# jmschrei/PyPore

Measured on AMD Instinct MI355X. Metric: Msamples/sec segmented (SpeedyStatSplit, 10^8-sample trace); %HBM roofline, higher is better.
Workload: dtype int32/f64 (exact integer block sums of fp32 or int16 samples; decisions in fp64)

## Files before the change

### pypore_amd/csrc/poreseg.hip

```cpp
#include <hip/hip_runtime.h>

#include <algorithm>
#include <chrono>
#include <complex>
#include <cmath>
#include <cstdarg>
#include <cstdio>
#include <cstdlib>
#include <cstring>
#include <condition_variable>
#include <mutex>
#include <string>
#include <thread>
#include <tuple>
#include <vector>

#include "poreseg.h"
#include "seg_device.hpp"
#include "seg_align.hpp"
#include "seg_pairwise.hpp"
#include "seg_hmm.hpp"

using namespace ps;

// ... 150 lines not shown
    }
    return code;
}

#define HIP_TRY(ctx, expr)                                                                        \
    do {                                                                                          \
        hipError_t e_ = (expr);                                                                   \
        if (e_ != hipSuccess)                                                                     \
            return fail(ctx, PS_ERR_HIP, "%s failed: %s (%s:%d)", #expr, hipGetErrorString(e_), __FILE__, __LINE__); \
    } while (0)

struct FrontStream { std::mutex mu; hipStream_t s = nullptr; };
FrontStream g_front[16];
FrontStream *front_for(ps_ctx *ctx)
{
    if (ctx->device < 0 || ctx->device >= 16) return nullptr;
    FrontStream *f = &g_front[ctx->device];
    std::lock_guard<std::mutex> lk(f->mu);
    if (!f->s) {
#ifdef PS_DIAG
        int lo = 0, hi = 0;
        const char *pr = std::getenv("PORESEG_FRONT_PRIORITY");
        if (pr && std::atoi(pr) != 0 && hipDeviceGetStreamPriorityRange(&lo, &hi) == hipSuccess) {
            if (hipStreamCreateWithPriority(&f->s, hipStreamNonBlocking, hi) != hipSuccess) { f->s = nullptr; (void)hipGetLastError(); }
        }
#endif
        if (!f->s && hipStreamCreateWithFlags(&f->s, hipStreamNonBlocking) != hipSuccess) { f->s = nullptr; (void)hipGetLastError(); return nullptr; }
    }
    return f;
}

struct K0Chain {
    static constexpr int RING = 64;
    std::mutex mu;
    hipEvent_t ev[RING] = {};
    unsigned long long gen[RING];
    unsigned long long next = 0;
    bool made = false;
};
K0Chain g_chain[16];
int chain_enter(ps_ctx *ctx, int device, int max_in_flight, hipStream_t st, unsigned long long *ticket)
{
    K0Chain &c = g_chain[device & 15];
    std::lock_guard<std::mutex> lk(c.mu);
    if (!c.made) {
        for (int i = 0; i < K0Chain::RING; ++i) { HIP_TRY(ctx, hipEventCreateWithFlags(&c.ev[i], hipEventDisableTiming)); c.gen[i] = 0; }
        c.made = true;
    }
    const unsigned long long t = c.next++;
    *ticket = t;
    const int m = std::min(max_in_flight, K0Chain::RING / 2);
    if (t >= static_cast<unsigned long long>(m)) {
        const unsigned long long w = t - static_cast<unsigned long long>(m);
        if (c.gen[w % K0Chain::RING] == w + 1) HIP_TRY(ctx, hipStreamWaitEvent(st, c.ev[w % K0Chain::RING], 0));
    }
    return PS_OK;
}
int chain_publish(ps_ctx *ctx, int device, hipStream_t st, unsigned long long ticket)
{
    K0Chain &c = g_chain[device & 15];
    std::lock_guard<std::mutex> lk(c.mu);
    HIP_TRY(ctx, hipEventRecord(c.ev[ticket % K0Chain::RING], st));
    c.gen[ticket % K0Chain::RING] = ticket + 1;
    return PS_OK;
}
constexpr size_t SMALL_TAIL = 64 * 1024;
struct SmallLayout { unsigned long long status, work0, work1, work2, dense, stamp[12], life[9], qctl, qhead, tree_tail; AsmHeader hdr;
                     unsigned long long lat_ctl[6]; int lat_prog[LAT_D];
                     unsigned long long nt_cur; };

int make_cfg(ps_ctx *ctx, const void *d_samples, const ps_sample_format *fmt, int mw, int maxw, int W,
             double min_gain, DevCfg *c)
{
    if (!fmt) return fail(ctx, PS_ERR_ARG, "sample format is NULL");
    if (fmt->dtype != PS_DTYPE_F32 && fmt->dtype != PS_DTYPE_I16)
        return fail(ctx, PS_ERR_ARG, "unknown dtype %d", fmt->dtype);
    if (!(fmt->quantum > 0) || !std::isfinite(fmt->quantum))
        return fail(ctx, PS_ERR_ARG, "quantum must be positive and finite");
    c->samples = d_samples;
    c->dtype = fmt->dtype;
    c->off_counts = fmt->dtype == PS_DTYPE_F32 ? 0 : fmt->offset_counts;
    c->dc_counts = fmt->dtype == PS_DTYPE_F32 ? static_cast<double>(fmt->offset_counts) : 0.0;
    c->noise_k = ctx->noise_k;
    c->inv_q = static_cast<float>(1.0 / fmt->quantum);
    c->q = fmt->quantum;
    c->q2 = fmt->quantum * fmt->quantum;
    c->mw = mw; c->maxw = maxw; c->W = W; c->half = W / 2;
    c->min_gain = min_gain;
    c->mode = ctx->mode;
    c->prune = ctx->prune;
    c->lds_cap = std::max(1, std::min(W, ctx->lds_max_samples));
    c->bsum = nullptr; c->ev_info = nullptr; c->chunk_tot = nullptr; c->blk_mm = nullptr; c->grp = nullptr; c->bs_wide = 0;
    c->blk_cls = nullptr; c->cls_mm = nullptr; c->cls_kthr = 0;
    c->k0_unaligned = ctx->k0_unaligned;
    c->pre_c = nullptr; c->pre_c2 = nullptr;
    c->dbg = ctx->small.as<SmallLayout>()->stamp;
    c->nt_log = nullptr;
// ... 761 lines not shown
                                       ctx->bridges.as<int2>(), ctx->bmeta.as<int4>(), reinterpret_cast<unsigned *>(&sm->status),           \
                                       &sm->work0, static_cast<int>(n_ext), ctx->ext_list.as<int>(), ctx->bridge_ext.as<int2>(),           \
                                       ctx->ext_slot.as<int>(), slots_used, BR_MAX, ext_stride)
            if (wide) { if (f32) PS_EXT(PS_DTYPE_F32 | DT_WIDE); else PS_EXT(PS_DTYPE_I16 | DT_WIDE); }
            else      { if (f32) PS_EXT(PS_DTYPE_F32); else PS_EXT(PS_DTYPE_I16); }
#undef PS_EXT
            HIP_TRY(ctx, hipGetLastError());
        }
        ctx->counters[4] += static_cast<int64_t>(n_ext);
        slots_used += static_cast<int>(n_ext);
        items_cap += static_cast<int64_t>(n_ext) * ext_stride;
        const int64_t ts2 = total_len / mw + items_cap + 1;
        HIP_TRY(ctx, ctx->spine_items.reserve(static_cast<size_t>(items_cap) * sizeof(int4)));
        HIP_TRY(ctx, ctx->tree_jobs.reserve(static_cast<size_t>(items_cap) * sizeof(TreeJob)));
        HIP_TRY(ctx, ctx->tree_counts.reserve((static_cast<size_t>(items_cap) + (static_cast<size_t>(items_cap) >> GS_LOG) + 2) * sizeof(int32_t)));
        HIP_TRY(ctx, ctx->items.reserve(static_cast<size_t>(items_cap) * sizeof(Item)));
        HIP_TRY(ctx, ctx->item_pos.reserve((static_cast<size_t>(items_cap) + 1) * sizeof(int64_t)));
        HIP_TRY(ctx, ctx->tree_scratch.reserve(static_cast<size_t>(ts2) * sizeof(int32_t)));
        HIP_TRY(ctx, ctx->tree_spill.reserve(static_cast<size_t>(ts2) * sizeof(int2)));
    }
    ctx->counters[3] = hd.n_items;
    float ms = 0;
    if (ctx->timing >= 2 && nj && hipEventElapsedTime(&ms, ctx->ev[7], ctx->ev[0]) == hipSuccess) ctx->ms[6] = ms;
    if (ctx->timing >= 2 && nj && hipEventElapsedTime(&ms, ctx->ev[0], ctx->ev[6]) == hipSuccess) ctx->ms[0] = ms;
    if (ctx->timing >= 2 && nj && hipEventElapsedTime(&ms, ctx->ev[6], ctx->ev[1]) == hipSuccess) ctx->ms[5] = ms;
    if (ctx->timing >= 2 && hipEventElapsedTime(&ms, ctx->ev[1], ctx->ev[5]) == hipSuccess) ctx->ms[4] = ms;
    return rc;
}
int device_stitch_batch(ps_ctx *ctx, const DevCfg &cfg_in, int bs_mode, const int64_t *ev_start, const int64_t *ev_len, int32_t n_ev, int mw, int W,
                        int32_t *d_bounds, int64_t cap, int64_t *h_bounds_off, ps_segstat *d_stats,
                        std::chrono::steady_clock::time_point t_begin, bool digest_ready = false)
{
    const int rc = device_stitch_batch_(ctx, cfg_in, bs_mode, ev_start, ev_len, n_ev, mw, W, d_bounds, cap, h_bounds_off, d_stats, t_begin, digest_ready);
    ctx->chain_held = false;
    return rc;
}
}

namespace {
std::mutex g_probe_mu;
int g_unaligned_ok[16] = {-1, -1, -1, -1, -1, -1, -1, -1, -1, -1, -1, -1, -1, -1, -1, -1};
int k0_unaligned_probe(int device, hipStream_t st)
{
    std::lock_guard<std::mutex> lk(g_probe_mu);
    int &ok = g_unaligned_ok[device & 15];
    if (ok >= 0) return ok;
    ok = 0;
    unsigned char h[128];
    for (int i = 0; i < 128; ++i) h[i] = static_cast<unsigned char>(37 * i + 11);
    unsigned char *d = nullptr;
    unsigned *bad = nullptr;
    if (hipMalloc(&d, 256) != hipSuccess || hipMalloc(&bad, sizeof(unsigned)) != hipSuccess) { if (d) (void)hipFree(d); (void)hipGetLastError(); return ok; }
    unsigned hb = 1;
    if (hipMemcpyAsync(d, h, 128, hipMemcpyHostToDevice, st) == hipSuccess && hipMemsetAsync(bad, 0, sizeof(unsigned), st) == hipSuccess) {
        hipLaunchKernelGGL(k0_unaligned_probe_kernel<2>, dim3(1), dim3(64), 0, st, d, 16, bad);
        hipLaunchKernelGGL(k0_unaligned_probe_kernel<4>, dim3(1), dim3(64), 0, st, d, 16, bad);
        if (hipGetLastError() == hipSuccess && hipMemcpyAsync(&hb, bad, sizeof(unsigned), hipMemcpyDeviceToHost, st) == hipSuccess &&
            hipStreamSynchronize(st) == hipSuccess)
            ok = hb == 0 ? 1 : 0;
    }
    (void)hipFree(d); (void)hipFree(bad); (void)hipGetLastError();
    return ok;
}
}

#ifdef PS_DIAG
// ... 125 lines not shown
        ctx->n_cu = hipGetDeviceProperties(&prop, ctx->device) == hipSuccess ? prop.multiProcessorCount : 256;
    }
    HIP_TRY(ctx, hipStreamSynchronize(*st));
    HIP_TRY(ctx, hipStreamDestroy(*st));
    *st = nullptr;
    if (count <= 0) { HIP_TRY(ctx, hipStreamCreateWithFlags(st, hipStreamNonBlocking)); return PS_OK; }
    const int words = (ctx->n_cu + 31) / 32;
    std::vector<uint32_t> mask(static_cast<size_t>(words), invert ? 0xffffffffu : 0u);
    for (int k = 0; k < count; ++k) {
        const int b = first + k * std::max(1, stride);
        if (b < 0 || b >= ctx->n_cu) continue;
        if (invert) mask[b >> 5] &= ~(1u << (b & 31)); else mask[b >> 5] |= 1u << (b & 31);
    }
    if (ctx->n_cu & 31) mask[words - 1] &= (1u << (ctx->n_cu & 31)) - 1u;
    HIP_TRY(ctx, hipExtStreamCreateWithCUMask(st, static_cast<uint32_t>(words), mask.data()));
    return PS_OK;
}
#endif

int ps_set_option(ps_ctx *ctx, const char *name, int64_t value)
{
    if (!ctx || !name) return PS_ERR_ARG;
    const std::string n(name);
    if (n == "mode" && value >= 0 && value <= 2) ctx->mode = static_cast<int>(value);
    else if (n == "stitch_host") ctx->stitch_host = value != 0;
    else if (n == "prune") ctx->prune = value != 0;
    else if (n == "scan_bs") ctx->scan_bs = value != 0;
    else if (n == "near_tie_log" && value >= 0 && value <= (int64_t(1) << 30)) ctx->nt_cap = value;
    else if (n == "groups") ctx->groups = value != 0;
    else if (n == "tree_par") ctx->tree_par = value != 0;
    else if (n == "k0_waves" && value >= 0 && value <= 16) ctx->k0_waves = static_cast<int>(value);
    else if (n == "k0_shared") ctx->k0_shared = value != 0;
    else if (n == "k0_admit" && value >= 0) ctx->k0_admit = static_cast<int>(value);
    else if (n == "bridge_ext" && (value == 0 || value == 1)) ctx->bridge_ext_on = static_cast<int>(value);
    else if (n == "lat_help" && value >= 0 && value <= 2) ctx->lat_help = static_cast<int>(value);
    else if (n == "shared_device" && value >= 0 && value <= 4096) {
        const bool sh = value > 1;
        ctx->k0_waves = sh ? 1 : 0;
        ctx->lat_help = sh ? 0 : 1;
        ctx->k0_admit = value > 3 ? 3 : 0;
    }
    else if (n == "hmm_bp_budget" && value >= 1) ctx->hmm_bp_budget = value;
    else if (n == "hmm_fb_budget" && value >= 1) ctx->hmm_fb_budget = value;
    else if (n == "pairwise_budget" && value >= 1) ctx->pw_budget = value;
    else if (n == "hmm_expect_lds") ctx->hmm_expect_lds = value != 0;
    else if (n == "single_pass") ctx->single_pass = value != 0;
    else if (n == "gather_fused") ctx->gather_fused = value != 0;
    else if (n == "download_by_kernel") ctx->download_by_kernel = value != 0;
    else if (n == "debug") ctx->debug = value != 0;
    else if (n == "k0_unaligned") ctx->k0_unaligned = value != 0 ? k0_unaligned_probe(ctx->device, ctx->stream) : 0;
    else if (n == "slots_pct" && value >= 1 && value <= 100) ctx->slots_pct = static_cast<int>(value);
    else if (n == "tree_jobs_per_wave" && value >= 0 && value <= 1024) ctx->tree_jobs_per_wave = static_cast<int>(value);
    else if (n == "noise_k_ppm" && value >= 0) ctx->noise_k = static_cast<float>(static_cast<double>(value) * 1.0e-6);
#ifdef PS_DIAG
    else if (n == "dbg_phase" && value >= 0 && value <= 2) ctx->dbg_phase = static_cast<int>(value);
    else if (n == "dbg_k0_nogrp") ctx->dbg_k0_nogrp = value != 0;
    else if (n == "cu_mask" && ctx->own_stream)
        return diag_mask_stream(ctx, &ctx->stream, static_cast<int>(value & 0xfff), static_cast<int>((value >> 12) & 0xfff),
                                static_cast<int>((value >> 24) & 0xff), ((value >> 32) & 1) != 0);
    else if (n == "k0_sets" && value >= 2 && value <= 4) ctx->k0_sets = static_cast<int>(value);
    else if (n == "scan_lds_pad" && value >= 0 && value <= 65536) ctx->scan_lds_pad = static_cast<int>(value);
    else if (n == "rep_eval" && value >= 1) ctx->rep_eval = static_cast<int>(value);
    else if (n == "rep_stage" && value >= 1) ctx->rep_stage = static_cast<int>(value);
    else if (n == "rep_sum" && value >= 1) ctx->rep_sum = static_cast<int>(value);
#endif
    else if (n == "bridge_budget" && value >= 1 && value <= BR_MAX) ctx->bridge_budget = static_cast<int>(value);
// ... 671 lines not shown
        kk = std::max(-2147483000.0, std::min(2147483000.0, kk));
        long long k = static_cast<long long>(kk);
        while (k > -2147483000LL && !(static_cast<double>(k - 1) * q < threshold)) --k;
        while (k < 2147483000LL && static_cast<double>(k) * q < threshold) ++k;
        kthr = static_cast<int>(k);
    }
    hipLaunchKernelGGL(trace_setup_kernel, dim3(1), dim3(256), 0, ctx->stream, reinterpret_cast<unsigned long long *>(ctx->small.p),
                       static_cast<int>(sizeof(SmallLayout) / sizeof(unsigned long long)), ctx->det_cand.as<long long>(),
                       static_cast<long long>(n), static_cast<long long>(nb_total));
    HIP_TRY(ctx, hipGetLastError());
    cfg.grp = ctx->groups ? ctx->grp.p : nullptr;
    cfg.blk_mm = d_stats ? ctx->blk_mm.as<int>() : nullptr;
    cfg.blk_cls = ctx->blk_cls.as<unsigned char>();
    cfg.cls_mm = ctx->cls_mm.as<int2>();
    cfg.cls_kthr = kthr;
    if (ctx->n_cu <= 0) {
        hipDeviceProp_t prop;
        ctx->n_cu = hipGetDeviceProperties(&prop, ctx->device) == hipSuccess ? prop.multiProcessorCount : 256;
    }
    {
        const unsigned k0_full = static_cast<unsigned>((nb_pad / K0_WB + K0_WAVES - 1) / K0_WAVES);
        const unsigned k0_per_cu = static_cast<unsigned>(ctx->k0_waves) * (f32 ? 1u : 2u);
        const unsigned k0_grid = ctx->k0_waves > 0 ? std::min(k0_full, k0_per_cu * static_cast<unsigned>(ctx->n_cu) * (4u / K0_WAVES)) : k0_full;
        const int64_t *d_ev = ctx->det_cand.as<int64_t>();
        if (ctx->k0_admit > 0) {
            const int grc = chain_enter(ctx, ctx->device, ctx->k0_admit, ctx->stream, &ctx->chain_ticket);
            if (grc) return grc;
        }
#define PS_K0T(DTV) hipLaunchKernelGGL((blocksum_kernel<DTV, 2>), dim3(k0_grid), dim3(64 * K0_WAVES), 0, ctx->stream, cfg, d_ev, d_ev + 1, d_ev + 2, 1, n, \
                                     ctx->bsum.p, ctx->ev_info.as<int4>(), ctx->chunk_mabs.as<int4>(), reinterpret_cast<unsigned *>(&sm->status),          \
                                     const_cast<uint4 *>(static_cast<const uint4 *>(cfg.grp)))
        if (f32) PS_K0T(PS_DTYPE_F32); else PS_K0T(PS_DTYPE_I16);
#undef PS_K0T
        HIP_TRY(ctx, hipGetLastError());
        if (ctx->k0_admit > 0) { const int crc = chain_publish(ctx, ctx->device, ctx->stream, ctx->chain_ticket); if (crc) return crc; }
    }
    std::vector<int> tics;
    unsigned st = 0;
    rc = detect_edges(ctx, cfg, n, threshold, true, tics, &st);
    if (rc) return rc;
    if (st & ST_WIDE_RANGE) { ctx->counters[7] = 3; const int r2 = two_calls(); ctx->counters[7] = 3; return r2; }
    rc = events_from_edges(ctx, cfg, n, tics, threshold, min_duration, min_current, h_starts, h_lengths, ev_cap, n_events_out);
    if (rc) return rc;
    const int32_t n_ev = static_cast<int32_t>(*n_events_out);
    if (n_ev == 0) { ctx->nt_seen = 0; return PS_OK; }
    for (int e = 0; e < n_ev; ++e)
        if (h_lengths[e] > 0x7fffffff - 2LL * W - 16) return fail(ctx, PS_ERR_ARG, "event %d length %lld out of range", e, static_cast<long long>(h_lengths[e]));
    cfg.bsum = ctx->bsum.p;
    cfg.blk_cls = nullptr;
    rc = device_stitch_batch(ctx, cfg, 1, h_starts, h_lengths, n_ev, mw, W, d_bounds, cap, h_bounds_off, d_stats, t_begin, true);
    if (rc == RC_FALLBACK || rc == RC_WIDE) {
        return ps_segment_events(ctx, d_samples, fmt, h_starts, h_lengths, n_ev, params, d_bounds, cap, h_bounds_off, d_stats, nullptr);
    }
    if (rc == PS_OK) nt_keep(ctx, h_starts, h_lengths, n_ev);
    else ctx->nt_seen = -1;
    return rc;
}

int ps_get_near_ties(const ps_ctx *ctx, ps_near_tie *out, int32_t cap, int64_t *n_out)
{
    if (!ctx || !n_out || cap < 0 || (cap > 0 && !out)) return PS_ERR_ARG;
    if (ctx->nt_seen < 0) { *n_out = PS_NT_NOT_COUNTED; return PS_OK; }
    if (ctx->nt_seen > ctx->nt_call_cap) { *n_out = PS_NT_INCOMPLETE; return PS_OK; }
    if (ctx->nt_seen == 0) { *n_out = 0; return PS_OK; }
    std::vector<NtRec> rec(static_cast<size_t>(ctx->nt_seen));
    if (hipSetDevice(ctx->device) != hipSuccess ||
        hipMemcpyAsync(rec.data(), static_cast<const char *>(ctx->nt_log.p) + offsetof(NtLog, rec), rec.size() * sizeof(NtRec), hipMemcpyDeviceToHost,
// ... 3 lines not shown
    const size_t ne = ctx->nt_ev_start.size();
    std::vector<int32_t> ord(ne);
    for (size_t e = 0; e < ne; ++e) ord[e] = static_cast<int32_t>(e);
    std::stable_sort(ord.begin(), ord.end(), [&](int32_t a, int32_t b) { return st[a] < st[b]; });
    std::vector<int64_t> reach(ne);
    for (size_t i = 0; i < ne; ++i) reach[i] = std::max(i ? reach[i - 1] : INT64_MIN, st[ord[i]] + ln[ord[i]]);
    std::vector<ps_near_tie> sites;
    for (const NtRec &r : rec) {
        const int64_t g = r.start, ge = r.start + r.len;
        size_t i = static_cast<size_t>(std::upper_bound(ord.begin(), ord.end(), g, [&](int64_t v, int32_t e) { return v < st[e]; }) - ord.begin());
        while (i > 0 && reach[i - 1] >= ge) {
            const int32_t e = ord[--i];
            if (st[e] <= g && ge <= st[e] + ln[e]) {
                const int32_t ws = static_cast<int32_t>(g - st[e]);
                sites.push_back({e, ws, static_cast<int32_t>(ge - st[e]), r.split < 0 ? -1 : ws + r.split});
            }
        }
    }
    auto key = [](const ps_near_tie &a) { return std::make_tuple(a.event, a.window_start, a.window_end, a.split); };
    std::sort(sites.begin(), sites.end(), [&](const ps_near_tie &a, const ps_near_tie &b) { return key(a) < key(b); });
    sites.erase(std::unique(sites.begin(), sites.end(), [&](const ps_near_tie &a, const ps_near_tie &b) { return key(a) == key(b); }),
                sites.end());
    *n_out = static_cast<int64_t>(sites.size());
    if (sites.size() > static_cast<size_t>(cap)) return PS_ERR_CAPACITY;
    std::copy(sites.begin(), sites.end(), out);
    return PS_OK;
}

int ps_get_timings(const ps_ctx *ctx, double *ms, int32_t n_ms, int64_t *counters, int32_t n_counters)
{
    if (!ctx) return PS_ERR_ARG;
    for (int i = 0; i < n_ms && ms; ++i) ms[i] = i < 8 ? ctx->ms[i] : 0.0;
    for (int i = 0; i < n_counters && counters; ++i) counters[i] = i < 14 ? ctx->counters[i] : 0;
    return PS_OK;
}

const int64_t *ps_counters(const ps_ctx *ctx) { return ctx ? ctx->counters : nullptr; }

int ps_synth_trace(ps_ctx *ctx, void *d_out, int32_t dtype, int64_t n, uint64_t seed,
                   const int64_t *h_seg_end, const int32_t *h_level_counts, int64_t nseg)
{
    if (!ctx) return PS_ERR_ARG;
    if (!d_out || n < 0 || nseg < 1 || !h_seg_end || !h_level_counts) return fail(ctx, PS_ERR_ARG, "bad argument");
    if (h_seg_end[nseg - 1] < n) return fail(ctx, PS_ERR_ARG, "segment table does not cover n");
    HIP_TRY(ctx, hipSetDevice(ctx->device));
    const size_t b1 = static_cast<size_t>(nseg) * sizeof(int64_t), b2 = static_cast<size_t>(nseg) * sizeof(int32_t);
    HIP_TRY(ctx, ctx->tree_scratch.reserve(b1 + b2));
    char *d = ctx->tree_scratch.as<char>();
    HIP_TRY(ctx, hipMemcpyAsync(d, h_seg_end, b1, hipMemcpyHostToDevice, ctx->stream));
    HIP_TRY(ctx, hipMemcpyAsync(d + b1, h_level_counts, b2, hipMemcpyHostToDevice, ctx->stream));
    HIP_TRY(ctx, hipStreamSynchronize(ctx->stream));
    hipLaunchKernelGGL(synth_kernel, dim3(4096), dim3(256), 0, ctx->stream, d_out, dtype, n,
                       static_cast<unsigned long long>(seed), reinterpret_cast<const int64_t *>(d),
                       reinterpret_cast<const int32_t *>(d + b1), nseg);
    HIP_TRY(ctx, hipGetLastError());
    HIP_TRY(ctx, hipStreamSynchronize(ctx->stream));
    return PS_OK;
}

namespace {
int filter_order_n(ps_ctx *ctx, const DevCfg &cfg, int64_t n, int order, double wn, double *d_out)
{
    typedef std::complex<double> cd;
    static const double poles[FILT_MAXORD + 1][4][2] = {
        {{0, 0}}, {{-0.9999999999999998, 0.0}},
        {{-0.8660254037844384, 0.4999999999999999}},
// ... 790 lines not shown
```

### pypore_amd/csrc/seg_bs.hpp

```cpp
#pragma once
#include <type_traits>

namespace ps {

constexpr int BS_WIDE = 16384;
enum : unsigned { ST_WIDE_RANGE = 16u };
constexpr int BS_CHUNK = 128;
constexpr int BS_CHUNK_LOG = 7;
constexpr int BS_MAXCH = 64;
constexpr int BSW_LIM = 1 << 23;
template <int DT> constexpr bool bs_wide() { return (DT & DT_WIDE) != 0; }
__device__ __forceinline__ long long i64_of(int lo, int hi) { return (static_cast<long long>(hi) << 32) | static_cast<unsigned>(lo); }
__device__ __forceinline__ double d_of_i64(long long x)
{
    return fma(static_cast<double>(static_cast<int>(x >> 32)), 4294967296.0, static_cast<double>(static_cast<unsigned>(x)));
}
__device__ __forceinline__ unsigned long long u64_of(unsigned lo, unsigned hi) { return (static_cast<unsigned long long>(hi) << 32) | lo; }
__device__ __forceinline__ int bs8_s1(uint2 v) { return static_cast<int>(v.y) >> 7; }
__device__ __forceinline__ unsigned long long bs8_s2(uint2 v) { return u64_of(v.x, v.y & 0x7fu); }
__device__ __forceinline__ double bs8_s2_biased(uint2 v) { return __hiloint2double(static_cast<int>((v.y & 0x7fu) | 0x43300000u), static_cast<int>(v.x)); }
constexpr double BS_BIAS = 4503599627370496.0;
__device__ __forceinline__ uint2 bs8_pack(int e1, unsigned long long e2)
{
    return make_uint2(static_cast<unsigned>(e2), (static_cast<unsigned>(e1) << 7) | static_cast<unsigned>(e2 >> 32));
// ... 105 lines not shown
    PS_OCT_STEPS(PS_STEP)
#undef PS_STEP
    return x;
}
__device__ __forceinline__ int oct_allmin(int x)
{
#define PS_STEP(CTRL) { x = min(x, dpp_mov<CTRL, 0xf>(0x7fffffff, x)); }
    PS_OCT_STEPS(PS_STEP)
#undef PS_STEP
    return x;
}
__device__ __forceinline__ float oct_allmaxf(float x)
{
#define PS_STEP(CTRL) { x = __uint_as_float(max(__float_as_uint(x), static_cast<unsigned>(dpp_mov<CTRL, 0xf>(0, static_cast<int>(__float_as_uint(x)))))); }
    PS_OCT_STEPS(PS_STEP)
#undef PS_STEP
    return x;
}
__device__ __forceinline__ float pmaxf(float a, float b) { return __int_as_float(max(__float_as_int(a), __float_as_int(b))); }
__device__ __forceinline__ int oct_first(int x, int lane)
{
    const int q = __builtin_amdgcn_update_dpp(0, x, 0x00, 0xf, 0xf, true);
    const int s = __builtin_amdgcn_update_dpp(0, q, 0x114, 0xf, 0xf, true);
    return (lane & 4) ? s : q;
}

#ifndef PS_K0_AMP
#define PS_K0_AMP 2
#endif
#ifndef PS_K0_TRIM
#define PS_K0_TRIM 1
#endif
#ifndef PS_K0_MINW
#define PS_K0_MINW 4
#endif
constexpr int K0_BPT = 4;
constexpr int K0_WB = 64 * K0_BPT;
#ifndef PS_K0_WAVES
#define PS_K0_WAVES 4
#endif
#ifndef PS_K0_PKF32
#define PS_K0_PKF32 1
#endif
#ifndef PS_K0_PK16
#define PS_K0_PK16 1
#endif
#ifndef PS_K0_PRIO
#define PS_K0_PRIO 0
#endif
constexpr int K0_WAVES = PS_K0_WAVES;
__host__ __device__ inline long long k0_padded_blocks(long long nb_total) { return (nb_total + 1 + K0_WB - 1) / K0_WB * K0_WB; }

__device__ __forceinline__ void k0_lds_ready() { asm volatile("s_waitcnt lgkmcnt(0)" ::: "memory"); __builtin_amdgcn_wave_barrier(); }
__device__ __forceinline__ void k0_lds_done() { __builtin_amdgcn_wave_barrier(); asm volatile("" ::: "memory"); }

template <int DT> struct K0Rec { int s1; unsigned s2; unsigned long long s2w; int ymin, ymax; };
template <int DT> struct K0Gen { K0Rec<DT> r; int m; unsigned bad; };

template <int DT>
__device__ __forceinline__ void k0_block_sums(const int (&y)[8], K0Rec<DT> &r)
{
    constexpr bool WIDE = bs_wide<DT>();
    r.s1 = 0; r.s2 = 0; r.s2w = 0;
#pragma unroll
    for (int q = 0; q < 8; ++q) {
        r.s1 += y[q];
        if constexpr (WIDE) r.s2w += static_cast<unsigned long long>(static_cast<long long>(y[q]) * static_cast<long long>(y[q]));
// ... 139 lines not shown
        for (int q = 0; q < 5; ++q) v[q] = q4[q];
        const bool odd = (a & 2u) != 0;
        const int om = c.off_counts - m;
#pragma unroll
        for (int q = 0; q < 4; ++q) {
            const int w = odd ? static_cast<int>((static_cast<unsigned>(v[q]) >> 16) | (static_cast<unsigned>(v[q + 1]) << 16)) : v[q];
            y[2 * q] = static_cast<int>(static_cast<short>(w & 0xffff)) + om;
            y[2 * q + 1] = (w >> 16) + om;
        }
        k0_block_sums<DT>(y, r);
    } else {
#pragma unroll
        for (int q = 0; q < 8; ++q) y[q] = q < cnt ? load_count<DT>(c, base + i0 + q, bad) - m : 0;
        k0_block_sums<DT>(y, r);
        r.ymin = r.ymax = y[0];
#pragma unroll
        for (int q = 1; q < 8; ++q)
            if (q < cnt) { r.ymin = min(r.ymin, y[q]); r.ymax = max(r.ymax, y[q]); }
    }
    if (b == 0) ev_info[e] = make_int4(m, 0, static_cast<int>(ev_boff[e] & 0xffffffffLL), static_cast<int>(ev_boff[e] >> 32));
    out.bad = bad;
    return out;
}

struct K0Src { int e; int fast; long long b_first; int64_t base; };
template <int A> struct K0Vec;
template <> struct K0Vec<2> { typedef int type __attribute__((ext_vector_type(4), aligned(2))); };
template <> struct K0Vec<4> { typedef int type __attribute__((ext_vector_type(4), aligned(4))); };
template <int A> __device__ __forceinline__ int4 k0_load16(const char *p)
{
    const typename K0Vec<A>::type v = *reinterpret_cast<const typename K0Vec<A>::type *>(p);
    return make_int4(v.x, v.y, v.z, v.w);
}
template <int A>
__global__ void k0_unaligned_probe_kernel(const unsigned char *buf, int n_off, unsigned *bad)
{
    const int o = threadIdx.x;
    if (o >= n_off) return;
    const int4 v = k0_load16<A>(reinterpret_cast<const char *>(buf) + o * A);
    const unsigned char *q = buf + o * A;
    unsigned w[4];
    for (int k = 0; k < 4; ++k) w[k] = q[4 * k] | (q[4 * k + 1] << 8) | (q[4 * k + 2] << 16) | (static_cast<unsigned>(q[4 * k + 3]) << 24);
    if (static_cast<unsigned>(v.x) != w[0] || static_cast<unsigned>(v.y) != w[1] || static_cast<unsigned>(v.z) != w[2] || static_cast<unsigned>(v.w) != w[3])
        atomicOr(bad, 1u);
}

template <int DT, int NS = 2>
__global__ __launch_bounds__(64 * K0_WAVES, (NS > 2 ? 2 : PS_K0_MINW)) void blocksum_kernel(DevCfg c, const int64_t *__restrict__ ev_start, const int64_t *__restrict__ ev_len,
                                                                const int64_t *__restrict__ ev_boff, int n_ev, int64_t n_samples, void *bs_out,
                                                                int4 *ev_info, int4 *chunk_tot, unsigned *status, uint4 *grp_out)
{
    constexpr bool WIDE = bs_wide<DT>();
    constexpr int LIM = WIDE ? BSW_LIM : BS_WIDE;
    constexpr int ES = static_cast<int>(sizeof(typename Raw<DT>::type));
    constexpr int NV = 8 * ES / 16;
    __shared__ int4 tr[K0_WAVES][K0_WB];
    const int lane = threadIdx.x & 63;
    const int wave = uni(static_cast<int>(threadIdx.x >> 6));
    const long long nwv = static_cast<long long>(gridDim.x) * K0_WAVES;
    long long wv = static_cast<long long>(blockIdx.x) * K0_WAVES + wave;
    const long long nb_total = ev_boff[n_ev];
    const long long n_wb = nb_total / K0_WB + 1;
    if (wv >= n_wb) return;
#if PS_K0_PRIO
    __builtin_amdgcn_s_setprio(PS_K0_PRIO);
#endif
    unsigned bad = 0;
    int4 *mine = tr[wave];
    auto classify = [&](long long wb0, int e_lo) -> K0Src {
        K0Src s;
        const long long gfirst = min(wb0, nb_total - 1);
        int lo = e_lo, hi = n_ev - 1;
        while (lo < hi) {
            const int mid = (lo + hi + 1) >> 1;
            if (ev_boff[mid] <= gfirst) lo = mid; else hi = mid - 1;
        }
        s.e = lo;
        s.b_first = wb0 - ev_boff[lo];
        s.base = ev_start[lo];
        const int64_t len_f = ev_len[lo];
        s.fast = wb0 + K0_WB <= ev_boff[lo + 1] && 8 * (s.b_first + K0_WB) <= len_f && nb_total > 0;
        if (!c.k0_unaligned && ((reinterpret_cast<uintptr_t>(c.samples) + static_cast<uintptr_t>((s.base + 8 * s.b_first) * ES)) & 15u) != 0) s.fast = 0;
        return s;
    };
    using raw_t = typename Raw<DT>::type;
    auto issue = [&](const K0Src &s, int4 (&raw)[K0_BPT][NV], raw_t &first) {
        const char *pb = s.fast ? static_cast<const char *>(c.samples) + (s.base + 8 * s.b_first) * ES : static_cast<const char *>(bs_out);
        first = *reinterpret_cast<const raw_t *>(s.fast ? static_cast<const char *>(c.samples) + s.base * ES : static_cast<const char *>(bs_out));
        const unsigned lo = static_cast<unsigned>(lane) * (8u * ES);
#pragma unroll
        for (int k = 0; k < K0_BPT; ++k)
#pragma unroll
            for (int v = 0; v < NV; ++v) raw[k][v] = k0_load16<ES>(pb + (lo + static_cast<unsigned>(k * 64 * 8 * ES + 16 * v)));
    };
    auto process = [&](auto fast_tag, const long long wb0, const K0Src &src, const int4 (&raw)[K0_BPT][NV], const raw_t first) {
    constexpr bool FAST = decltype(fast_tag)::value;
    const int e_first = src.e;
    int ymn_all = 0x7fffffff, ymx_all = -0x7fffffff - 1;
    auto put = [&](int k, const K0Rec<DT> &r) {
        if (PS_K0_TRIM) { ymn_all = min(ymn_all, r.ymin); ymx_all = max(ymx_all, r.ymax); }
        else if (r.ymax >= LIM || r.ymin <= -LIM) bad |= ST_WIDE_RANGE;
        if constexpr (WIDE) mine[64 * k + lane] = make_int4(r.s1, max(-r.ymin, r.ymax), static_cast<int>(r.s2w), static_cast<int>(r.s2w >> 32));
        else mine[64 * k + lane] = make_int4(r.s1, static_cast<int>(r.s2), (r.ymin & 0xffff) | (r.ymax << 16), 0);
    };
    if constexpr (FAST) {
        const int m = to_count<DT>(c, first, bad);
        const float mf = static_cast<float>(m);
        unsigned nz = 0;
        const bool look = sdt(DT) == PS_DTYPE_F32 && (WIDE || m > 8388607 - LIM || m < -8388607 + LIM);
        constexpr bool PK16 = sdt(DT) == PS_DTYPE_I16 && !WIDE && PS_K0_PK16;
        const int k0raw = m - c.off_counts;
        const int k0pk = (k0raw & 0xffff) | (k0raw << 16);
#pragma unroll
        for (int k = 0; k < K0_BPT; ++k) {
            int y[8];
            K0Rec<DT> r;
            if constexpr (PK16) {
                k0_block_sums_pk16<DT>(raw[k][0], k0pk, r);
            } else if constexpr (sdt(DT) == PS_DTYPE_F32 && !WIDE && PS_K0_PKF32) {
                k0_block_sums_pkf32<DT>(raw[k], c.inv_q, mf, nz, r);
                asm volatile("" : "+v"(nz));
            } else {
            k0_offsets<DT>(c, raw[k], m, mf, nz, y);
            asm volatile("" : "+v"(nz));
            k0_block_sums<DT>(y, r);
            }
            if (!PS_K0_TRIM && look) {
                const int ka = m + r.ymin, kb = m + r.ymax;
                if (max(ka < 0 ? -ka : ka, kb < 0 ? -kb : kb) >= 8388608) bad |= ST_OFF_GRID;
            }
            put(k, r);
            __builtin_amdgcn_sched_barrier(0);
        }
        if (PS_K0_TRIM && look) {
            const int ka = m + ymn_all, kb = m + ymx_all;
            if (max(ka < 0 ? -ka : ka, kb < 0 ? -kb : kb) >= 8388608) bad |= ST_OFF_GRID;
        }
        if (nz) bad |= ST_OFF_GRID;
        if (src.b_first + lane == 0) ev_info[e_first] = make_int4(m, 0, static_cast<int>(ev_boff[e_first] & 0xffffffffLL), static_cast<int>(ev_boff[e_first] >> 32));
    } else {
#pragma unroll 1
        for (int k = 0; k < K0_BPT; ++k) {
            const K0Gen<DT> g = k0_block_general<DT>(bs_cold(c), ev_start, ev_len, ev_boff, n_samples, wb0 + 64 * k + lane, nb_total, e_first, ev_info);
            bad |= g.bad;
            if (sdt(DT) == PS_DTYPE_F32) {
                const int ka = g.m + g.r.ymin, kb = g.m + g.r.ymax;
                if (max(ka < 0 ? -ka : ka, kb < 0 ? -kb : kb) >= 8388608) bad |= ST_OFF_GRID;
            }
            put(k, g.r);
        }
    }
    if (PS_K0_TRIM && (ymx_all >= LIM || ymn_all <= -LIM)) bad |= ST_WIDE_RANGE;
    k0_lds_ready();
    int4 t[K0_BPT];
#pragma unroll
    for (int j = 0; j < K0_BPT; ++j) t[j] = mine[K0_BPT * lane + j];
    const long long gb4 = wb0 + K0_BPT * lane;
    const long long chunk = (wb0 >> BS_CHUNK_LOG) + (lane >> 5);
    if constexpr (WIDE) {
        long long e1[K0_BPT], e2[K0_BPT];
        long long r1 = 0, r2 = 0;
        int yabs = 0;
#pragma unroll
        for (int j = 0; j < K0_BPT; ++j) {
            e1[j] = r1; e2[j] = r2;
            r1 += t[j].x; r2 += i64_of(t[j].z, t[j].w);
            yabs = max(yabs, t[j].y);
        }
        const long long i1 = half_incl_scan_i64(r1), i2 = half_incl_scan_i64(r2);
        const long long x1 = i1 - r1, x2 = i2 - r2;
        int4 *bs = static_cast<int4 *>(bs_out) + gb4;
#pragma unroll
// ... 111 lines not shown
            for (int j = 0; j < K0_BPT; ++j) {
                p1 += t[j].x;
                p2 += static_cast<double>(static_cast<unsigned>(t[j].y));
                const int jb = jb0 + j + 1;
                const int d1x = 32 * p1 - jb * S1g;
                const double d2 = fma(k1, static_cast<double>(d1x), fma(static_cast<double>(jb), k2, p2));
                m1 = max(m1, d1x < 0 ? -d1x : d1x);
                m2 = fmax(m2, fabs(d2));
            }
            const int gmn = oct_allmin(mmn), gmx = oct_allmax(mmx);
            m1 = oct_allmax(m1);
            const float m2f = oct_allmaxf(static_cast<float>(m2) * 1.000001f);
            const float mug = static_cast<float>(S1g) * (1.0f / static_cast<float>(BS_GRP_SAMPLES));
            const float Mg = fmaxf(static_cast<float>(gmx) - mug, mug - static_cast<float>(gmn)) * 1.000001f + 0.01f;
            const float D1 = (static_cast<float>(m1) * (1.0f / 32.0f) + 2.0f * static_cast<float>(gmx - gmn)) * 1.000001f;
            const float D2 = fmaf(2.0f * Mg, Mg, m2f) * 1.000001f;
            if ((lane & 7) == 0) grp_out[gb4 >> BS_GRP_LOG] = make_uint4(ent[0].x, ent[0].y, __float_as_uint(D1), __float_as_uint(D2));
        }
#endif
        yabs = half_max_i32(yabs);
        if ((lane & 31) == 31) {
            const unsigned long long tot2 = (static_cast<unsigned long long>(static_cast<unsigned>(ihi)) << 16) + static_cast<unsigned>(ilo);
            chunk_tot[chunk] = make_int4(i1, yabs, static_cast<int>(tot2), static_cast<int>(tot2 >> 32));
        }
    }
    k0_lds_done();
    };
    int4 raw[NS][K0_BPT][NV];
    raw_t first[NS];
    K0Src src[NS];
    unsigned long long general = 0;
    int it = 0;
    const long long wv0 = wv;
    auto retire = [&](const int4 (&rw)[K0_BPT][NV], const raw_t fs) {
#pragma unroll
        for (int k = 0; k < K0_BPT; ++k)
#pragma unroll
            for (int v = 0; v < NV; ++v) asm volatile("" :: "v"(rw[k][v].x), "v"(rw[k][v].y), "v"(rw[k][v].z), "v"(rw[k][v].w));
        asm volatile("" :: "v"(fs));
    };
    int e_hint = 0;
#pragma unroll
    for (int q = 0; q < NS - 1; ++q) {
        const long long wq = wv + q * nwv;
        if (wq < n_wb) { src[q] = classify(wq * K0_WB, e_hint); e_hint = src[q].e; }
        else { src[q] = src[0]; src[q].fast = 0; }
        issue(src[q], raw[q], first[q]);
    }
    bool last = false;
#pragma unroll 1
    while (!last) {
#pragma unroll
        for (int q = 0; q < NS; ++q) {
            if (last) break;
            constexpr int NSm1 = NS - 1;
            const int f = (q + NSm1) % NS;
            const long long wn = wv + static_cast<long long>(NSm1) * nwv;
            if (wn < n_wb) { src[f] = classify(wn * K0_WB, e_hint); e_hint = src[f].e; } else src[f].fast = 0;
            issue(src[f], raw[f], first[f]);
            if (src[q].fast) process(std::true_type{}, wv * K0_WB, src[q], raw[q], first[q]);
            else { general |= 1ull << min(it, 63); retire(raw[q], first[q]); }
            if (wv + nwv >= n_wb) last = true;
            else { wv += nwv; ++it; }
        }
    }
    if (general) {
        int e_lo = 0;
        it = 0;
#pragma unroll 1
        for (wv = wv0; wv < n_wb; wv += nwv, ++it) {
            if (it < 63 && !((general >> it) & 1ull)) continue;
            const K0Src sg = classify(wv * K0_WB, e_lo);
            e_lo = sg.e;
            if (!sg.fast) process(std::false_type{}, wv * K0_WB, sg, raw[0], first[0]);
        }
    }
    if (bad) atomicOr(status, bad);
}

struct BsEval { float g; f2 lg; f2 r; f2 u; bool okL, okR; };

__device__ __forceinline__ BsEval bs_eval(double a1d, double a2, double b1d, double b2, int nl, int nr, f2 cc, float vfloor)
{
    const double DL = fma(static_cast<double>(nl), a2, -(a1d * a1d));
    const double DR = fma(static_cast<double>(nr), b2, -(b1d * b1d));
    const f2 D = {static_cast<float>(DL), static_cast<float>(DR)};
    const f2 nv = {static_cast<float>(nl), static_cast<float>(nr)};
    const f2 r = {__builtin_amdgcn_rcpf(nv.x), __builtin_amdgcn_rcpf(nv.y)};
    const f2 u = D * r * r;
    const f2 lgu = {__builtin_amdgcn_logf(u.x), __builtin_amdgcn_logf(u.y)};
    BsEval o;
    o.lg = lgu - cc;
    o.r = r;
    o.u = u;
    o.okL = u.x >= vfloor;
    o.okR = u.y >= vfloor;
    const f2 t = nv * o.lg;
// ... 972 lines not shown
```

Measured before the change: 504,500.

## Harden K0 admission chain, add audit, and restructure blocksum load pipeline

Makes the K0 admission chain wait on a condition variable until the predecessor ticket is published, and abandons tickets when a launch fails. It also adds optional event-span auditing that reports peak concurrency through the counters. In the blocksum kernel, loads now use wave-uniform global address-space pointers with 4 KiB-aligned bases, and the unrolled ring loop is rewritten as compile-time-indexed steps. Retire now uses an explicit s_waitcnt vmcnt instead of register-pinning asm, and the minimum wave count rises from 4 to 5. The host wait can stall submitting threads, and the hand-written vmcnt assumes a fixed number of outstanding loads.

```diff
diff --git a/pypore_amd/csrc/poreseg.hip b/pypore_amd/csrc/poreseg.hip
--- a/pypore_amd/csrc/poreseg.hip
+++ b/pypore_amd/csrc/poreseg.hip
@@ -206,27 +206,54 @@
 
 struct K0Chain {
     static constexpr int RING = 64;
+    static constexpr size_t AUDIT_CAP = 16384;
     std::mutex mu;
+    std::condition_variable cv;
     hipEvent_t ev[RING] = {};
     unsigned long long gen[RING];
+    unsigned long long taken[RING];
+    bool recorded[RING];
     unsigned long long next = 0;
+    unsigned long long unguarded = 0;
     bool made = false;
+    int audit = 0;
+    std::vector<std::pair<hipEvent_t, hipEvent_t>> spans;
+    std::vector<hipEvent_t> spare;
 };
 K0Chain g_chain[16];
 int chain_enter(ps_ctx *ctx, int device, int max_in_flight, hipStream_t st, unsigned long long *ticket)
 {
     K0Chain &c = g_chain[device & 15];
-    std::lock_guard<std::mutex> lk(c.mu);
+    std::unique_lock<std::mutex> lk(c.mu);
     if (!c.made) {
-        for (int i = 0; i < K0Chain::RING; ++i) { HIP_TRY(ctx, hipEventCreateWithFlags(&c.ev[i], hipEventDisableTiming)); c.gen[i] = 0; }
+        for (int i = 0; i < K0Chain::RING; ++i) {
+            HIP_TRY(ctx, hipEventCreateWithFlags(&c.ev[i], hipEventDisableTiming));
+            c.gen[i] = 0; c.taken[i] = 0; c.recorded[i] = false;
+        }
         c.made = true;
     }
     const unsigned long long t = c.next++;
     *ticket = t;
+    c.taken[t % K0Chain::RING] = t + 1;
     const int m = std::min(max_in_flight, K0Chain::RING / 2);
     if (t >= static_cast<unsigned long long>(m)) {
         const unsigned long long w = t - static_cast<unsigned long long>(m);
-        if (c.gen[w % K0Chain::RING] == w + 1) HIP_TRY(ctx, hipStreamWaitEvent(st, c.ev[w % K0Chain::RING], 0));
+        const int s = static_cast<int>(w % K0Chain::RING);
+        const bool there = c.cv.wait_for(lk, std::chrono::seconds(2), [&] { return c.taken[s] != w + 1 || c.gen[s] == w + 1; });
+        if (!there) ++c.unguarded;
+        else if (c.taken[s] == w + 1 && c.recorded[s]) {
+            const hipError_t e = hipStreamWaitEvent(st, c.ev[s], 0);
+            if (e != hipSuccess) {
+                c.gen[t % K0Chain::RING] = t + 1; c.recorded[t % K0Chain::RING] = false;
+                c.cv.notify_all();
+                return fail(ctx, PS_ERR_HIP, "hipStreamWaitEvent (K0 admission) failed: %s", hipGetErrorString(e));
+            }
+        }
+    }
+    if (c.audit && c.spans.size() < K0Chain::AUDIT_CAP && t == c.spans.size()) {
+        hipEvent_t a = nullptr, b = nullptr;
+        if (hipEventCreate(&a) == hipSuccess && hipEventCreate(&b) == hipSuccess && hipEventRecord(a, st) == hipSuccess) c.spans.emplace_back(a, b);
+        else { (void)hipGetLastError(); c.audit = 0; }
     }
     return PS_OK;
 }
@@ -234,9 +261,53 @@
 {
     K0Chain &c = g_chain[device & 15];
     std::lock_guard<std::mutex> lk(c.mu);
-    HIP_TRY(ctx, hipEventRecord(c.ev[ticket % K0Chain::RING], st));
-    c.gen[ticket % K0Chain::RING] = ticket + 1;
-    return PS_OK;
+    const int s = static_cast<int>(ticket % K0Chain::RING);
+    if (c.audit && ticket < c.spans.size()) (void)hipEventRecord(c.spans[ticket].second, st);
+    const hipError_t e = hipEventRecord(c.ev[s], st);
+    c.gen[s] = ticket + 1;
+    c.recorded[s] = e == hipSuccess;
+    c.cv.notify_all();
+    if (e != hipSuccess) return fail(ctx, PS_ERR_HIP, "hipEventRecord (K0 admission) failed: %s", hipGetErrorString(e));
+    return PS_OK;
+}
+void chain_abandon(int device, unsigned long long ticket)
+{
+    K0Chain &c = g_chain[device & 15];
+    std::lock_guard<std::mutex> lk(c.mu);
+    const int s = static_cast<int>(ticket % K0Chain::RING);
+    if (c.taken[s] == ticket + 1 && c.gen[s] != ticket + 1) { c.gen[s] = ticket + 1; c.recorded[s] = false; }
+    c.cv.notify_all();
+}
+void chain_audit(int device, int mode)
+{
+    K0Chain &c = g_chain[device & 15];
+    std::lock_guard<std::mutex> lk(c.mu);
+    if (mode == 2) {
+        for (auto &sp : c.spans) { (void)hipEventDestroy(sp.first); (void)hipEventDestroy(sp.second); }
+        c.spans.clear();
+        c.next = 0; c.unguarded = 0;
+        for (int i = 0; i < K0Chain::RING; ++i) { c.gen[i] = 0; c.taken[i] = 0; c.recorded[i] = false; }
+    }
+    c.audit = mode != 0;
+}
+void chain_audit_read(int device, int64_t *out)
+{
+    K0Chain &c = g_chain[device & 15];
+    std::lock_guard<std::mutex> lk(c.mu);
+    out[0] = -1; out[1] = static_cast<int64_t>(c.spans.size()); out[2] = static_cast<int64_t>(c.unguarded);
+    if (c.spans.empty()) return;
+    std::vector<std::pair<float, int>> edge;
+    for (const auto &sp : c.spans) {
+        float a = 0.0f, b = 0.0f;
+        if (hipEventSynchronize(sp.second) != hipSuccess || hipEventElapsedTime(&a, c.spans[0].first, sp.first) != hipSuccess ||
+            hipEventElapsedTime(&b, c.spans[0].first, sp.second) != hipSuccess) { (void)hipGetLastError(); return; }
+        edge.emplace_back(a, 1); edge.emplace_back(b, -1);
+    }
+    std::sort(edge.begin(), edge.end(), [](const std::pair<float, int> &x, const std::pair<float, int> &y) {
+        return x.first < y.first || (x.first == y.first && x.second < y.second); });
+    int64_t cur = 0, hw = 0;
+    for (const auto &e : edge) { cur += e.second; hw = std::max(hw, cur); }
+    out[0] = hw;
 }
 constexpr size_t SMALL_TAIL = 64 * 1024;
 struct SmallLayout { unsigned long long status, work0, work1, work2, dense, stamp[12], life[9], qctl, qhead, tree_tail; AsmHeader hdr;
@@ -1064,6 +1135,7 @@
                         std::chrono::steady_clock::time_point t_begin, bool digest_ready = false)
 {
     const int rc = device_stitch_batch_(ctx, cfg_in, bs_mode, ev_start, ev_len, n_ev, mw, W, d_bounds, cap, h_bounds_off, d_stats, t_begin, digest_ready);
+    if (ctx->chain_held) chain_abandon(ctx->device, ctx->chain_ticket);
     ctx->chain_held = false;
     return rc;
 }
@@ -1255,6 +1327,7 @@
     else if (n == "k0_waves" && value >= 0 && value <= 16) ctx->k0_waves = static_cast<int>(value);
     else if (n == "k0_shared") ctx->k0_shared = value != 0;
     else if (n == "k0_admit" && value >= 0) ctx->k0_admit = static_cast<int>(value);
+    else if (n == "k0_audit" && value >= 0 && value <= 2) chain_audit(ctx->device, static_cast<int>(value));
     else if (n == "bridge_ext" && (value == 0 || value == 1)) ctx->bridge_ext_on = static_cast<int>(value);
     else if (n == "lat_help" && value >= 0 && value <= 2) ctx->lat_help = static_cast<int>(value);
     else if (n == "shared_device" && value >= 0 && value <= 4096) {
@@ -1992,7 +2065,10 @@
                                      const_cast<uint4 *>(static_cast<const uint4 *>(cfg.grp)))
         if (f32) PS_K0T(PS_DTYPE_F32); else PS_K0T(PS_DTYPE_I16);
 #undef PS_K0T
-        HIP_TRY(ctx, hipGetLastError());
+        if (const hipError_t le = hipGetLastError(); le != hipSuccess) {
+            if (ctx->k0_admit > 0) chain_abandon(ctx->device, ctx->chain_ticket);
+            return fail(ctx, PS_ERR_HIP, "blocksum_kernel launch failed: %s", hipGetErrorString(le));
+        }
         if (ctx->k0_admit > 0) { const int crc = chain_publish(ctx, ctx->device, ctx->stream, ctx->chain_ticket); if (crc) return crc; }
     }
     std::vector<int> tics;
@@ -2062,6 +2138,11 @@
     if (!ctx) return PS_ERR_ARG;
     for (int i = 0; i < n_ms && ms; ++i) ms[i] = i < 8 ? ctx->ms[i] : 0.0;
     for (int i = 0; i < n_counters && counters; ++i) counters[i] = i < 14 ? ctx->counters[i] : 0;
+    if (counters && n_counters > 14) {
+        int64_t a[3];
+        chain_audit_read(ctx->device, a);
+        for (int i = 14; i < n_counters && i < 17; ++i) counters[i] = a[i - 14];
+    }
     return PS_OK;
 }
 
diff --git a/pypore_amd/csrc/seg_bs.hpp b/pypore_amd/csrc/seg_bs.hpp
--- a/pypore_amd/csrc/seg_bs.hpp
+++ b/pypore_amd/csrc/seg_bs.hpp
@@ -161,7 +161,7 @@
 #define PS_K0_TRIM 1
 #endif
 #ifndef PS_K0_MINW
-#define PS_K0_MINW 4
+#define PS_K0_MINW 5
 #endif
 constexpr int K0_BPT = 4;
 constexpr int K0_WB = 64 * K0_BPT;
@@ -367,6 +367,17 @@
     const typename K0Vec<A>::type v = *reinterpret_cast<const typename K0Vec<A>::type *>(p);
     return make_int4(v.x, v.y, v.z, v.w);
 }
+typedef const __attribute__((address_space(1))) char *k0_gptr;
+__device__ __forceinline__ k0_gptr k0_global_uni(const char *p)
+{
+    return reinterpret_cast<k0_gptr>(static_cast<uintptr_t>(uni(static_cast<long long>(reinterpret_cast<uintptr_t>(p)))));
+}
+template <int A> __device__ __forceinline__ int4 k0_load16(k0_gptr p)
+{
+    typedef const __attribute__((address_space(1))) typename K0Vec<A>::type *vptr;
+    const typename K0Vec<A>::type v = *reinterpret_cast<vptr>(p);
+    return make_int4(v.x, v.y, v.z, v.w);
+}
 template <int A>
 __global__ void k0_unaligned_probe_kernel(const unsigned char *buf, int n_off, unsigned *bad)
 {
@@ -424,11 +435,14 @@
         first = *reinterpret_cast<const raw_t *>(s.fast ? static_cast<const char *>(c.samples) + s.base * ES : static_cast<const char *>(bs_out));
         const unsigned lo = static_cast<unsigned>(lane) * (8u * ES);
 #pragma unroll
-        for (int k = 0; k < K0_BPT; ++k)
-#pragma unroll
-            for (int v = 0; v < NV; ++v) raw[k][v] = k0_load16<ES>(pb + (lo + static_cast<unsigned>(k * 64 * 8 * ES + 16 * v)));
+        for (int k = 0; k < K0_BPT; ++k) {
+            constexpr int ROW = 64 * 8 * ES;
+            const k0_gptr pk = k0_global_uni(pb + (k * ROW) / 4096 * 4096);
+#pragma unroll
+            for (int v = 0; v < NV; ++v) raw[k][v] = k0_load16<ES>(pk + (lo + static_cast<unsigned>((k * ROW) % 4096 + 16 * v)));
+        }
     };
-    auto process = [&](auto fast_tag, const long long wb0, const K0Src &src, const int4 (&raw)[K0_BPT][NV], const raw_t first) {
+    auto process = [&](auto fast_tag, const long long wb0, const K0Src &src, const int4 (&raw)[K0_BPT][NV], const raw_t first) __attribute__((always_inline)) {
     constexpr bool FAST = decltype(fast_tag)::value;
     const int e_first = src.e;
     int ymn_all = 0x7fffffff, ymx_all = -0x7fffffff - 1;
@@ -472,7 +486,7 @@
             if (max(ka < 0 ? -ka : ka, kb < 0 ? -kb : kb) >= 8388608) bad |= ST_OFF_GRID;
         }
         if (nz) bad |= ST_OFF_GRID;
-        if (src.b_first + lane == 0) ev_info[e_first] = make_int4(m, 0, static_cast<int>(ev_boff[e_first] & 0xffffffffLL), static_cast<int>(ev_boff[e_first] >> 32));
+        if (src.b_first == 0 && lane == 0) ev_info[e_first] = make_int4(m, 0, static_cast<int>(ev_boff[e_first] & 0xffffffffLL), static_cast<int>(ev_boff[e_first] >> 32));
     } else {
 #pragma unroll 1
         for (int k = 0; k < K0_BPT; ++k) {
@@ -650,12 +664,10 @@
     unsigned long long general = 0;
     int it = 0;
     const long long wv0 = wv;
-    auto retire = [&](const int4 (&rw)[K0_BPT][NV], const raw_t fs) {
-#pragma unroll
-        for (int k = 0; k < K0_BPT; ++k)
-#pragma unroll
-            for (int v = 0; v < NV; ++v) asm volatile("" :: "v"(rw[k][v].x), "v"(rw[k][v].y), "v"(rw[k][v].z), "v"(rw[k][v].w));
-        asm volatile("" :: "v"(fs));
+    auto retire = [&]() {
+        constexpr int YOUNGER = (NS - 1) * (K0_BPT * NV + 1);
+        static_assert(YOUNGER < 64, "vmcnt is a six-bit counter");
+        asm volatile("s_waitcnt vmcnt(%0)" :: "n"(YOUNGER) : "memory");
     };
     int e_hint = 0;
 #pragma unroll
@@ -665,22 +677,26 @@
         else { src[q] = src[0]; src[q].fast = 0; }
         issue(src[q], raw[q], first[q]);
     }
-    bool last = false;
+    auto step = [&](auto q_tag) __attribute__((always_inline)) -> bool {
+        constexpr int Q = decltype(q_tag)::value;
+        constexpr int NSm1 = NS - 1;
+        constexpr int F = (Q + NSm1) % NS;
+        const long long wn = wv + static_cast<long long>(NSm1) * nwv;
+        if (wn < n_wb) { src[F] = classify(wn * K0_WB, e_hint); e_hint = src[F].e; } else src[F].fast = 0;
+        issue(src[F], raw[F], first[F]);
+        if (src[Q].fast) process(std::true_type{}, wv * K0_WB, src[Q], raw[Q], first[Q]);
+        else { general |= 1ull << min(it, 63); retire(); }
+        if (wv + nwv >= n_wb) return true;
+        wv += nwv; ++it;
+        return false;
+    };
 #pragma unroll 1
-    while (!last) {
-#pragma unroll
-        for (int q = 0; q < NS; ++q) {
-            if (last) break;
-            constexpr int NSm1 = NS - 1;
-            const int f = (q + NSm1) % NS;
-            const long long wn = wv + static_cast<long long>(NSm1) * nwv;
-            if (wn < n_wb) { src[f] = classify(wn * K0_WB, e_hint); e_hint = src[f].e; } else src[f].fast = 0;
-            issue(src[f], raw[f], first[f]);
-            if (src[q].fast) process(std::true_type{}, wv * K0_WB, src[q], raw[q], first[q]);
-            else { general |= 1ull << min(it, 63); retire(raw[q], first[q]); }
-            if (wv + nwv >= n_wb) last = true;
-            else { wv += nwv; ++it; }
-        }
+    for (;;) {
+        if (step(std::integral_constant<int, 0>{})) break;
+        if (step(std::integral_constant<int, 1>{})) break;
+        if constexpr (NS > 2) { if (step(std::integral_constant<int, 2 % NS>{})) break; }
+        if constexpr (NS > 3) { if (step(std::integral_constant<int, 3 % NS>{})) break; }
+        static_assert(NS >= 2 && NS <= 4, "two to four register sets");
     }
     if (general) {
         int e_lo = 0;
```

After: 502,900. About the same (-0.3%).
